# MasterBin-IIAU/UNINEXT

Hardware: NVIDIA H100
Metric: msdeformattn_fwd_bwd_gsamples_per_s (higher is better)
Workload: dtype f32

## Files before the change

### uninext_b200/csrc/msda_common.cuh

```cuda
#pragma once

#include <cuda_bf16.h>
#include <cuda_runtime.h>
#include <stdint.h>

namespace msda {

constexpr int kMaxLevels = 8;
constexpr unsigned kFullMask = 0xffffffffu;

__device__ __forceinline__ void pdl_launch_dependents() { asm volatile("griddepcontrol.launch_dependents;" ::: "memory"); }
__device__ __forceinline__ void pdl_wait_primary() { asm volatile("griddepcontrol.wait;" ::: "memory"); }

struct TapGeom {
    float lh, lw;
    int r0, r1;
    int dw;
    unsigned mask;
};

__device__ __forceinline__ TapGeom tap_geometry(float x, float y, int H, int W, int start) {
    TapGeom g;
    const float h_im = __fadd_rn(__fmul_rn(y, (float)H), -0.5f);
    const float w_im = __fadd_rn(__fmul_rn(x, (float)W), -0.5f);
    const bool inside = (h_im > -1.f) && (w_im > -1.f) && (h_im < (float)H) && (w_im < (float)W);
    const float hf = floorf(h_im), wf = floorf(w_im);
    g.lh = h_im - hf;
    g.lw = w_im - wf;
    int h0 = inside ? (int)hf : 0;
    int w0 = inside ? (int)wf : 0;
    const int h1 = h0 + 1, w1 = w0 + 1;
    unsigned m = 0;
    if (inside) {
        const bool t = h0 >= 0, b = h1 <= H - 1, l = w0 >= 0, r = w1 <= W - 1;
        m = (unsigned)(t && l) | ((unsigned)(t && r) << 1) | ((unsigned)(b && l) << 2) | ((unsigned)(b && r) << 3);
    }
    g.mask = m;
    const int ch0 = max(h0, 0), ch1 = min(h1, H - 1), cw0 = max(w0, 0), cw1 = min(w1, W - 1);
    g.r0 = start + ch0 * W + cw0;
    g.r1 = start + ch1 * W + cw0;
    g.dw = cw1 - cw0;
    return g;
}

template <typename T, int VEC> struct RowVec;

template <> struct RowVec<float, 4> {
    static constexpr int kElems = 4;
    __device__ static __forceinline__ void load(const float *p, float (&v)[4]) {
        const float4 t = __ldg(reinterpret_cast<const float4 *>(p));
        v[0] = t.x; v[1] = t.y; v[2] = t.z; v[3] = t.w;
    }
    __device__ static __forceinline__ void store(float *p, const float (&v)[4]) {
        *reinterpret_cast<float4 *>(p) = make_float4(v[0], v[1], v[2], v[3]);
    }
};

template <> struct RowVec<float, 8> {
    static constexpr int kElems = 8;
    __device__ static __forceinline__ void load(const float *p, float (&v)[8]) {
        const float4 a = __ldg(reinterpret_cast<const float4 *>(p)), b = __ldg(reinterpret_cast<const float4 *>(p) + 1);
        v[0] = a.x; v[1] = a.y; v[2] = a.z; v[3] = a.w; v[4] = b.x; v[5] = b.y; v[6] = b.z; v[7] = b.w;
    }
    __device__ static __forceinline__ void store(float *p, const float (&v)[8]) {
        reinterpret_cast<float4 *>(p)[0] = make_float4(v[0], v[1], v[2], v[3]);
        reinterpret_cast<float4 *>(p)[1] = make_float4(v[4], v[5], v[6], v[7]);
    }
};

template <> struct RowVec<__nv_bfloat16, 4> {
    static constexpr int kElems = 4;
    __device__ static __forceinline__ void load(const __nv_bfloat16 *p, float (&v)[4]) {
        const uint2 t = __ldg(reinterpret_cast<const uint2 *>(p));
        v[0] = __uint_as_float(t.x << 16); v[1] = __uint_as_float(t.x & 0xffff0000u);
        v[2] = __uint_as_float(t.y << 16); v[3] = __uint_as_float(t.y & 0xffff0000u);
    }
    __device__ static __forceinline__ void store(__nv_bfloat16 *p, const float (&v)[4]) {
        const __nv_bfloat162 a = __floats2bfloat162_rn(v[0], v[1]), b = __floats2bfloat162_rn(v[2], v[3]);
        *reinterpret_cast<uint2 *>(p) = make_uint2(*reinterpret_cast<const unsigned *>(&a),
                                                   *reinterpret_cast<const unsigned *>(&b));
    }
};

template <> struct RowVec<__nv_bfloat16, 8> {
    static constexpr int kElems = 8;
    __device__ static __forceinline__ void load(const __nv_bfloat16 *p, float (&v)[8]) {
        const uint4 t = __ldg(reinterpret_cast<const uint4 *>(p));
        const unsigned u[4] = {t.x, t.y, t.z, t.w};
#pragma unroll
        for (int i = 0; i < 4; ++i) {
            v[2 * i] = __uint_as_float(u[i] << 16);
            v[2 * i + 1] = __uint_as_float(u[i] & 0xffff0000u);
        }
    }
    __device__ static __forceinline__ void store(__nv_bfloat16 *p, const float (&v)[8]) {
        unsigned u[4];
#pragma unroll
        for (int i = 0; i < 4; ++i) {
            const __nv_bfloat162 h = __floats2bfloat162_rn(v[2 * i], v[2 * i + 1]);
            u[i] = *reinterpret_cast<const unsigned *>(&h);
        }
        *reinterpret_cast<uint4 *>(p) = make_uint4(u[0], u[1], u[2], u[3]);
    }
};

__device__ __forceinline__ void red_add_v4(float *addr, float a, float b, float c, float d) {
    asm volatile("red.global.add.v4.f32 [%0], {%1, %2, %3, %4};" ::"l"(addr), "f"(a), "f"(b), "f"(c), "f"(d) : "memory");
}

__device__ __forceinline__ void red_add_bf16x4(__nv_bfloat16 *addr, float a, float b, float c, float d) {
    const __nv_bfloat162 lo = __floats2bfloat162_rn(a, b), hi = __floats2bfloat162_rn(c, d);
    asm volatile("red.global.add.noftz.v2.bf16x2 [%0], {%1, %2};" ::"l"(addr), "r"(*reinterpret_cast<const unsigned *>(&lo)),
                 "r"(*reinterpret_cast<const unsigned *>(&hi)) : "memory");
}

__device__ __forceinline__ void red_add_mixed(bool to_bf16, __nv_bfloat16 *a16, bool to_f32, float *a32, float a, float b,
                                              float c, float d) {
    const __nv_bfloat162 lo = __floats2bfloat162_rn(a, b), hi = __floats2bfloat162_rn(c, d);
    asm volatile(
        "{\n\t.reg .pred p16, p32;\n\t"
        "setp.ne.b32 p16, %0, 0;\n\t"
        "setp.ne.b32 p32, %1, 0;\n\t"
        "@p16 red.global.add.noftz.v2.bf16x2 [%2], {%3, %4};\n\t"
        "@p32 red.global.add.v4.f32 [%5], {%6, %7, %8, %9};\n\t}"
        ::"r"((unsigned)to_bf16), "r"((unsigned)to_f32), "l"(a16), "r"(*reinterpret_cast<const unsigned *>(&lo)),
          "r"(*reinterpret_cast<const unsigned *>(&hi)), "l"(a32), "f"(a), "f"(b), "f"(c), "f"(d) : "memory");
}

}
```

### uninext_b200/csrc/msda_region.cuh

```cuda
#pragma once

#include "msda_tiled.cuh"

namespace msda {

constexpr int kRegionEdge = 8;
constexpr int kRegionHalo = 2;
constexpr int kRegionSlots = 96;
constexpr int kRegionWinRows = 1024;
constexpr int kRegionStageRows = 384;
constexpr int kRegionEntries = kRegionSlots * 16 * 4;
constexpr int kRegionTapCtas = 2;
constexpr int kRegionGvCtas = 3;
constexpr int kRegionIterSlots = kTiledWarps * 4;

using RegionTapStage = TapStage<4, 16, true>;

constexpr size_t region_tap_smem_bytes() { return (size_t)kTiledWarps * RegionTapStage::kBytes; }

constexpr size_t region_gv_smem_bytes() {
    static_assert(kRegionEntries <= 0x10000, "entry indices are u16");
    return (size_t)kRegionEntries * (4 + 2 + 2) + (size_t)kRegionSlots * 128 + (size_t)kRegionWinRows * 4;
}

#ifdef MSDA_REGION_PHASE_CLOCKS
constexpr int kRegionSpans = 4;
__device__ unsigned long long *g_region_clocks;
__device__ int g_region_knockout;
#define MSDA_REGION_CLOCK_INIT long long region_clk = clock64()
#define MSDA_REGION_CLOCK(span)                                                                  \
    if (threadIdx.x == 0) {                                                                      \
        const long long now = clock64();                                                         \
        g_region_clocks[blockIdx.x * kRegionSpans + (span)] += (unsigned long long)(now - region_clk); \
        region_clk = now;                                                                        \
    }
#define MSDA_REGION_KEEP_RED(bit) (!(g_region_knockout & (bit)))
#else
#define MSDA_REGION_CLOCK_INIT
#define MSDA_REGION_CLOCK(span)
#define MSDA_REGION_KEEP_RED(bit) true
#endif

#ifdef MSDA_REGION_COSCHED
__device__ unsigned long long *g_region_cosched[2];
__device__ __forceinline__ unsigned long long region_globaltimer() {
    unsigned long long t;
    asm volatile("mov.u64 %0, %%globaltimer;" : "=l"(t));
    return t;
}
#define MSDA_REGION_COSCHED_START(k)                                                               \
    if (threadIdx.x == 0) {                                                                        \
        unsigned smid;                                                                             \
        asm volatile("mov.u32 %0, %%smid;" : "=r"(smid));                                         \
        g_region_cosched[k][3 * blockIdx.x] = smid;                                                \
        g_region_cosched[k][3 * blockIdx.x + 1] = region_globaltimer();                            \
    }
#define MSDA_REGION_COSCHED_END(k)                                                                 \
    __syncthreads();                                                                               \
    if (threadIdx.x == 0) g_region_cosched[k][3 * blockIdx.x + 2] = region_globaltimer();
#else
#define MSDA_REGION_COSCHED_START(k)
#define MSDA_REGION_COSCHED_END(k)
#endif

struct RegionMap {
    int H[kMaxLevels], W[kMaxLevels], start[kMaxLevels];
    int Href, Wref, nry, nrx;
    int region;
    unsigned ntiles;
};

struct RegionTile {
    int b, m, nq, nwin;
    unsigned base_pair;
    int qy0[kMaxLevels], qx0[kMaxLevels], qny[kMaxLevels], qnx[kMaxLevels], qpre[kMaxLevels + 1];
    int wy0[kMaxLevels], wx0[kMaxLevels], wh[kMaxLevels], ww[kMaxLevels], wbase[kMaxLevels + 1];
};

__device__ __forceinline__ int region_first(int r, int n, int ref, int R) {
    const long long num = 2ll * r * n * R - ref;
    return num <= 0 ? 0 : (int)min((long long)n, (num + 2ll * ref - 1) / (2ll * ref));
}

template <int R, int HALO>
__global__ void __launch_bounds__(kTiledThreads, kRegionGvCtas)
msda_region_grad_value_pass(const float *__restrict__ grad_out, const int64_t *__restrict__ shapes,
                            const int64_t *__restrict__ lsi, const float *__restrict__ loc,
                            const float *__restrict__ attn, int N, int S, int M, int L, int Lq, int P, unsigned npairs,
                            float *__restrict__ grad_value)
{
    constexpr int D = 32, VEC = 4, LPR = D / VEC, GPW = 32 / LPR, LP_MAX = 16, NSL = LP_MAX / LPR;
    static_assert(GPW * kTiledWarps == kRegionIterSlots && kRegionSlots <= 256 && kRegionWinRows < 0xffff &&
                  kRegionSlots % kRegionIterSlots == 0, "entry layout");
    constexpr unsigned short kNoRow = 0xffff;

    __shared__ RegionMap rm;
    __shared__ RegionTile tl;
    __shared__ int wsum[kTiledWarps];
    __shared__ __align__(16) unsigned char slab_mem[kTiledWarps * TapSlab<LPR>::kBytes];
    extern __shared__ __align__(128) unsigned char region_dyn[];
    float *e_coef = reinterpret_cast<float *>(region_dyn);
    float4 *gstash = reinterpret_cast<float4 *>(e_coef + kRegionEntries);
    int *cnt = reinterpret_cast<int *>(gstash + kRegionSlots * LPR);
    unsigned short *e_row = reinterpret_cast<unsigned short *>(cnt + kRegionWinRows);
    unsigned short *s_idx = e_row + kRegionEntries;

    pdl_launch_dependents();
    MSDA_REGION_COSCHED_START(0);
    MSDA_REGION_CLOCK_INIT;
    if (threadIdx.x == 0) {
        int run = 0, href = 0, wref = 0;
        bool tiled = (Lq == S);
        for (int l = 0; l < L; ++l) {
            const int h = (int)shapes[2 * l], w = (int)shapes[2 * l + 1], st = (int)lsi[l];
            rm.H[l] = h; rm.W[l] = w; rm.start[l] = st;
            tiled = tiled && (st == run) && h > 0 && w > 0;
            run += h * w;
            href = max(href, h); wref = max(wref, w);
        }
        tiled = tiled && (run == S);
        rm.region = tiled ? 1 : 0;
        rm.Href = href; rm.Wref = wref;
        rm.nry = (href + R - 1) / R; rm.nrx = (wref + R - 1) / R;
        rm.ntiles = tiled ? (unsigned)N * (unsigned)M * (unsigned)(rm.nry * rm.nrx)
                          : (npairs + kRegionIterSlots - 1) / kRegionIterSlots;
    }
    __syncthreads();

    const int lane = threadIdx.x & 31, warp = threadIdx.x >> 5;
    const int sub = lane % LPR, grp = lane / LPR;
    const int LP = L * P;
    const unsigned row_elems = (unsigned)(M * D);
    TapSlab<LPR> slab(slab_mem + warp * TapSlab<LPR>::kBytes, grp);
    bool primary_done = false;
    for (unsigned tile = blockIdx.x; tile < rm.ntiles; tile += gridDim.x) {
        if (rm.region) {
            const int m = (int)(tile % (unsigned)M);
            const unsigned r = tile / (unsigned)M, per_b = (unsigned)(rm.nry * rm.nrx);
            const int reg = (int)(r % per_b), ry = reg / rm.nrx, rx = reg % rm.nrx;
            const int l = threadIdx.x;
            if (l < L) {
                const int H = rm.H[l], W = rm.W[l];
                const int y0 = region_first(ry, H, rm.Href, R), y1 = region_first(ry + 1, H, rm.Href, R);
                const int x0 = region_first(rx, W, rm.Wref, R), x1 = region_first(rx + 1, W, rm.Wref, R);
                tl.qy0[l] = y0; tl.qny[l] = y1 - y0; tl.qx0[l] = x0; tl.qnx[l] = x1 - x0;
                const int wy0 = max(0, (int)((long long)ry * R * H / rm.Href) - HALO);
                const int wy1 = min(H, (int)(((long long)(ry + 1) * R * H + rm.Href - 1) / rm.Href) + HALO);
                const int wx0 = max(0, (int)((long long)rx * R * W / rm.Wref) - HALO);
                const int wx1 = min(W, (int)(((long long)(rx + 1) * R * W + rm.Wref - 1) / rm.Wref) + HALO);
                tl.wy0[l] = wy0; tl.wh[l] = wy1 - wy0; tl.wx0[l] = wx0; tl.ww[l] = wx1 - wx0;
            }
            if (threadIdx.x == 0) { tl.m = m; tl.b = (int)(r / per_b); }
            __syncthreads();
            if (threadIdx.x == 0) {
                int nq = 0, nw = 0;
                for (int k = 0; k < L; ++k) {
                    tl.qpre[k] = nq; nq += tl.qny[k] * tl.qnx[k];
                    const int rows = tl.wh[k] * tl.ww[k];
                    if (nw + rows > kRegionWinRows) { tl.wh[k] = tl.ww[k] = 0; }
                    tl.wbase[k] = nw; nw += tl.wh[k] * tl.ww[k];
                }
                tl.qpre[L] = nq; tl.wbase[L] = nw;
                tl.nq = nq; tl.nwin = nw;
            }
        } else if (threadIdx.x == 0) {
            tl.base_pair = tile * kRegionIterSlots;
            tl.nq = (int)min((unsigned)kRegionIterSlots, npairs - tl.base_pair);
            tl.nwin = 0;
        }
        __syncthreads();
        for (int i = threadIdx.x; i < tl.nwin; i += kTiledThreads) cnt[i] = 0;
        __syncthreads();
        MSDA_REGION_CLOCK(0);

#pragma unroll 1
        for (int it = 0; it * kRegionIterSlots < tl.nq; ++it) {
            const int slot = it * kRegionIterSlots + warp * GPW + grp;
            const bool active = slot < tl.nq;
            unsigned pair = 0; int b = 0, m = 0;
            if (active) {
                if (rm.region) {
                    int l = 0;
                    while (l + 1 < L && slot >= tl.qpre[l + 1]) ++l;
                    const int k = slot - tl.qpre[l], y = tl.qy0[l] + k / tl.qnx[l], x = tl.qx0[l] + k % tl.qnx[l];
                    b = tl.b; m = tl.m;
                    pair = ((unsigned)b * (unsigned)Lq + (unsigned)(rm.start[l] + y * rm.W[l] + x)) * (unsigned)M + (unsigned)m;
                } else {
                    pair = tl.base_pair + (unsigned)slot;
                    m = (int)(pair % (unsigned)M);
                    b = (int)((pair / (unsigned)M) / (unsigned)Lq);
                }
            }
            const bool stash = rm.region && active && slot < kRegionSlots;

            float g[VEC] = {0.f, 0.f, 0.f, 0.f};
            if (active) RowVec<float, VEC>::load(grad_out + (size_t)pair * D + (size_t)sub * VEC, g);
            if (stash) gstash[slot * LPR + sub] = make_float4(g[0], g[1], g[2], g[3]);

            float4 tw[NSL];
            int2 tr[NSL];
#pragma unroll
            for (int k = 0; k < NSL; ++k) {
                const int s = sub + k * LPR;
                tw[k] = make_float4(0.f, 0.f, 0.f, 0.f);
                tr[k] = make_int2(0, 0);
                unsigned filed = 0;
                ushort4 rows4 = make_ushort4(kNoRow, kNoRow, kNoRow, kNoRow);
                float4 w4 = make_float4(0.f, 0.f, 0.f, 0.f);
                if (s < LP && active) {
                    const size_t t = (size_t)pair * LP + s;
                    const float2 xy = __ldg(reinterpret_cast<const float2 *>(loc) + t);
                    const float a = __ldg(attn + t);
                    const int l = s / P;
                    const TapGeom gm = tap_geometry(xy.x, xy.y, rm.H[l], rm.W[l], rm.start[l]);
                    w4 = masked_weights(gm, a);
                    tr[k] = make_int2(gm.r0, gm.r1 | (gm.dw << 31));
                    const unsigned nz = (unsigned)(w4.x != 0.f) | ((unsigned)(w4.y != 0.f) << 1) |
                                        ((unsigned)(w4.z != 0.f) << 2) | ((unsigned)(w4.w != 0.f) << 3);
                    if (stash) {
                        const int W = rm.W[l], o0 = gm.r0 - rm.start[l], o1 = gm.r1 - rm.start[l];
                        const int y0 = o0 / W, x0 = o0 - y0 * W, y1 = o1 / W;
                        const int wwl = tl.ww[l], whl = tl.wh[l];
                        const int ry0 = y0 - tl.wy0[l], ry1 = y1 - tl.wy0[l], rx0 = x0 - tl.wx0[l], rx1 = rx0 + gm.dw;
                        const unsigned iy0 = (unsigned)ry0 < (unsigned)whl, iy1 = (unsigned)ry1 < (unsigned)whl;
                        const unsigned ix0 = (unsigned)rx0 < (unsigned)wwl, ix1 = (unsigned)rx1 < (unsigned)wwl;
                        const unsigned inwin = (iy0 & ix0) | ((iy0 & ix1) << 1) | ((iy1 & ix0) << 2) | ((iy1 & ix1) << 3);
                        filed = inwin & nz;
                        const int w00 = tl.wbase[l] + ry0 * wwl + rx0, dhw = (y1 - y0) * wwl;
                        const int wr[4] = {w00, w00 + gm.dw, w00 + dhw, w00 + dhw + gm.dw};
#pragma unroll
                        for (int c = 0; c < 4; ++c)
                            if ((filed >> c) & 1u) atomicAdd(&cnt[wr[c]], 1);
                        rows4 = make_ushort4((filed & 1u) ? (unsigned short)wr[0] : kNoRow,
                                             (filed & 2u) ? (unsigned short)wr[1] : kNoRow,
                                             (filed & 4u) ? (unsigned short)wr[2] : kNoRow,
                                             (filed & 8u) ? (unsigned short)wr[3] : kNoRow);
                    }
                    tw[k] = make_float4((filed & 1u) ? 0.f : w4.x, (filed & 2u) ? 0.f : w4.y,
                                        (filed & 4u) ? 0.f : w4.z, (filed & 8u) ? 0.f : w4.w);
                }
                if (stash) {
                    const int e = (slot * LP_MAX + s) << 2;
                    *reinterpret_cast<ushort4 *>(e_row + e) = rows4;
                    *reinterpret_cast<float4 *>(e_coef + e) = w4;
                }
            }

            if (!primary_done) {
                pdl_wait_primary();
                primary_done = true;
            }
            const size_t slab_off = ((size_t)b * S * M + m) * D + (size_t)sub * VEC;
            float *gbase = grad_value + slab_off;
#pragma unroll
            for (int k = 0; k < NSL; ++k) {
                __syncwarp();
                slab.put(sub, tw[k], tr[k]);
                __syncwarp();
                const bool any = tw[k].x != 0.f || tw[k].y != 0.f || tw[k].z != 0.f || tw[k].w != 0.f;
                unsigned todo = (__ballot_sync(kFullMask, any) >> (grp * LPR)) & ((1u << LPR) - 1u);
                while (todo) {
                    const int j = __ffs(todo) - 1;
                    todo &= todo - 1u;
                    const float4 w4 = slab.weights(j);
                    const int2 rr = slab.rows(j);
                    const float w[4] = {w4.x, w4.y, w4.z, w4.w};
                    const unsigned dwo = (rr.y < 0) ? row_elems : 0u;
                    unsigned long long off[4];
                    off[0] = (unsigned long long)(unsigned)rr.x * row_elems;
                    off[1] = off[0] + dwo;
                    off[2] = (unsigned long long)(unsigned)(rr.y & 0x7fffffff) * row_elems;
                    off[3] = off[2] + dwo;
#pragma unroll
                    for (int c = 0; c < 4; ++c)
                        if (w[c] != 0.f && MSDA_REGION_KEEP_RED(1))
                            red_add_v4(gbase + off[c], w[c] * g[0], w[c] * g[1], w[c] * g[2], w[c] * g[3]);
                }
            }
        }

        const int nwin = tl.nwin;
        if (nwin > 0) {
            __syncthreads();
            MSDA_REGION_CLOCK(1);
            const int n = min(tl.nq, kRegionSlots) * LP_MAX * 4;
            {
                const int i0 = threadIdx.x * 4;
                int c[4], sum = 0;
#pragma unroll
                for (int q = 0; q < 4; ++q) { c[q] = (i0 + q < nwin) ? cnt[i0 + q] : 0; sum += c[q]; }
                int incl = sum;
#pragma unroll
                for (int d = 1; d < 32; d <<= 1) {
                    const int t = __shfl_up_sync(kFullMask, incl, d);
                    if (lane >= d) incl += t;
                }
                if (lane == 31) wsum[warp] = incl;
                __syncthreads();
                int run = incl - sum;
                for (int w = 0; w < warp; ++w) run += wsum[w];
#pragma unroll
                for (int q = 0; q < 4; ++q)
                    if (i0 + q < nwin) { cnt[i0 + q] = run; run += c[q]; }
            }
            static_assert(kRegionWinRows <= 4 * kTiledThreads, "scan covers 4 rows per thread");
            __syncthreads();
            for (int e = threadIdx.x; e < n; e += kTiledThreads) {
                const unsigned short r = e_row[e];
                if (r != kNoRow) s_idx[atomicAdd(&cnt[r], 1)] = (unsigned short)e;
            }
            __syncthreads();
            MSDA_REGION_CLOCK(2);

            const int b = tl.b, m = tl.m;
            for (int r = warp * GPW + grp; r < nwin; r += kRegionIterSlots) {
                const int beg = r ? cnt[r - 1] : 0, end = cnt[r];
                if (beg == end) continue;
                float4 acc = make_float4(0.f, 0.f, 0.f, 0.f);
#pragma unroll 4
                for (int i = beg; i < end; ++i) {
                    const int e = s_idx[i];
                    const float cf = e_coef[e];
                    const float4 gs = gstash[(e / (LP_MAX * 4)) * LPR + sub];
                    acc.x = fmaf(cf, gs.x, acc.x); acc.y = fmaf(cf, gs.y, acc.y);
                    acc.z = fmaf(cf, gs.z, acc.z); acc.w = fmaf(cf, gs.w, acc.w);
                }
                int l = 0;
                while (l + 1 < L && r >= tl.wbase[l + 1]) ++l;
                const int k = r - tl.wbase[l], y = tl.wy0[l] + k / tl.ww[l], x = tl.wx0[l] + k % tl.ww[l];
                const int row = rm.start[l] + y * rm.W[l] + x;
                if (MSDA_REGION_KEEP_RED(2))
                    red_add_v4(grad_value + (((size_t)b * S + row) * M + m) * D + (size_t)sub * VEC, acc.x, acc.y, acc.z, acc.w);
            }
        }
        __syncthreads();
        MSDA_REGION_CLOCK(nwin > 0 ? 3 : 1);
    }
    if (!primary_done) pdl_wait_primary();
    MSDA_REGION_COSCHED_END(0);
}

template <int R, int HALO>
__global__ void __launch_bounds__(kTiledThreads, kRegionTapCtas)
msda_bwd_region(const float *__restrict__ grad_out, const float *__restrict__ value,
                const int64_t *__restrict__ shapes, const int64_t *__restrict__ lsi,
                const float *__restrict__ loc, const float *__restrict__ attn,
                int N, int S, int M, int L, int Lq, int P, unsigned npairs, int tma,
                float *__restrict__ grad_loc, float *__restrict__ grad_attn)
{
    __shared__ WorkMap wm;
    __shared__ __align__(16) unsigned char slab_mem[kTiledWarps * TapSlab<8>::kBytes];
    __shared__ __align__(8) unsigned long long stage_bar[kTiledWarps * 2];
    extern __shared__ __align__(128) unsigned char stage_mem[];

    MSDA_REGION_COSCHED_START(1);
    if (tma)
        bwd_tiled_body<float, 4, 32, 16, true, false, false, true, false>(
            wm, slab_mem, stage_mem, stage_bar, grad_out, value, shapes, lsi, loc, attn, N, S, M, L, Lq, P, npairs, 0,
            nullptr, grad_loc, grad_attn, nullptr, 0);
    else
        bwd_tiled_body<float, 4, 32, 16, false, false, false, true, false>(
            wm, slab_mem, stage_mem, stage_bar, grad_out, value, shapes, lsi, loc, attn, N, S, M, L, Lq, P, npairs, 0,
            nullptr, grad_loc, grad_attn, nullptr, 0);
    MSDA_REGION_COSCHED_END(1);
    pdl_wait_primary();
}

struct RegionGrids {
    int gv, tap;
    size_t gv_smem;
    int gv_solo, tap_solo;
};

template <class GV, class TAP>
RegionGrids region_grids(GV gvk, size_t gv_smem, TAP tap, size_t tap_smem, int sms) {
    const auto occupancy = [](auto kern, size_t smem) {
        int per_sm = 0;
        if (cudaOccupancyMaxActiveBlocksPerMultiprocessor(&per_sm, kern, kTiledThreads, smem) != cudaSuccess || per_sm < 1)
            per_sm = 1;
        return per_sm;
    };
    const int gv_occ = occupancy(gvk, gv_smem), tap_occ = occupancy(tap, tap_smem);
    const RegionGrids solo = {gv_occ * sms, tap_occ * sms, gv_smem, gv_occ * sms, tap_occ * sms};
    int dev = 0, regs_sm = 0, smem_sm = 0, smem_optin = 0, reserved = 0, threads_sm = 0;
    cudaFuncAttributes ga{}, ta{};
    if (cudaGetDevice(&dev) != cudaSuccess ||
        cudaDeviceGetAttribute(&regs_sm, cudaDevAttrMaxRegistersPerMultiprocessor, dev) != cudaSuccess ||
        cudaDeviceGetAttribute(&smem_sm, cudaDevAttrMaxSharedMemoryPerMultiprocessor, dev) != cudaSuccess ||
        cudaDeviceGetAttribute(&smem_optin, cudaDevAttrMaxSharedMemoryPerBlockOptin, dev) != cudaSuccess ||
        cudaDeviceGetAttribute(&reserved, cudaDevAttrReservedSharedMemoryPerBlock, dev) != cudaSuccess ||
        cudaDeviceGetAttribute(&threads_sm, cudaDevAttrMaxThreadsPerMultiProcessor, dev) != cudaSuccess ||
        cudaFuncGetAttributes(&ga, gvk) != cudaSuccess || cudaFuncGetAttributes(&ta, tap) != cudaSuccess)
        return solo;
    constexpr int warps = kTiledThreads / 32;
    const auto regs = [](int per_thread) { return warps * ((per_thread * 32 + 255) / 256 * 256); };
    const auto smem = [&](const cudaFuncAttributes &a, size_t dyn) { return (long long)a.sharedSizeBytes + (long long)dyn + reserved; };
    for (int g = gv_occ; g >= 1; --g) {
        size_t dyn = gv_smem;
        if (g < gv_occ) {
            const long long over = (long long)smem_sm / (g + 1) + 1 - smem(ga, 0);
            dyn = (size_t)((over + 1023) / 1024 * 1024);
        }
        if ((long long)g * regs(ga.numRegs) + regs(ta.numRegs) <= regs_sm && (long long)dyn <= smem_optin &&
            g * smem(ga, dyn) + smem(ta, tap_smem) <= smem_sm && (g + 1) * kTiledThreads <= threads_sm) {
            if (dyn != gv_smem &&
                (cudaFuncSetAttribute(gvk, cudaFuncAttributeMaxDynamicSharedMemorySize, (int)dyn) != cudaSuccess ||
                 cudaFuncSetAttribute(gvk, cudaFuncAttributePreferredSharedMemoryCarveout,
                                      (int)cudaSharedmemCarveoutMaxShared) != cudaSuccess ||
                 occupancy(gvk, dyn) != g))
                return solo;
            return {g * sms, sms, dyn, solo.gv_solo, solo.tap_solo};
        }
    }
    return solo;
}

}
```

Baseline: 5.988.

## Replace shared-memory tap slab with warp shuffles and use 32-bit tile geometry

The grad_value kernel no longer stages each tap's weights and rows through a per-warp shared-memory slab. Each tap's scatter is now broadcast within its lane group by shuffles, inside the per-tap loop. This frees static shared memory and registers (tw/tr arrays) and drops the syncwarps. Tile-geometry arithmetic moves from 64-bit to 32-bit unsigned, guarded by a max-reference-size check, and TapGeom now carries clamped y/x coordinates so the integer divisions to recover them are gone. The carveout attribute is also now always set, which may change co-scheduling occupancy.

```diff
diff --git a/uninext_b200/csrc/msda_common.cuh b/uninext_b200/csrc/msda_common.cuh
--- a/uninext_b200/csrc/msda_common.cuh
+++ b/uninext_b200/csrc/msda_common.cuh
@@ -17,6 +17,7 @@
     int r0, r1;
     int dw;
     unsigned mask;
+    int y0, y1, x0;
 };
 
 __device__ __forceinline__ TapGeom tap_geometry(float x, float y, int H, int W, int start) {
@@ -40,6 +41,7 @@
     g.r0 = start + ch0 * W + cw0;
     g.r1 = start + ch1 * W + cw0;
     g.dw = cw1 - cw0;
+    g.y0 = ch0; g.y1 = ch1; g.x0 = cw0;
     return g;
 }
 
diff --git a/uninext_b200/csrc/msda_region.cuh b/uninext_b200/csrc/msda_region.cuh
--- a/uninext_b200/csrc/msda_region.cuh
+++ b/uninext_b200/csrc/msda_region.cuh
@@ -8,6 +8,7 @@
 constexpr int kRegionHalo = 2;
 constexpr int kRegionSlots = 96;
 constexpr int kRegionWinRows = 1024;
+constexpr int kRegionMaxRef = 1 << 15;
 constexpr int kRegionStageRows = 384;
 constexpr int kRegionEntries = kRegionSlots * 16 * 4;
 constexpr int kRegionTapCtas = 2;
@@ -78,8 +79,8 @@
 };
 
 __device__ __forceinline__ int region_first(int r, int n, int ref, int R) {
-    const long long num = 2ll * r * n * R - ref;
-    return num <= 0 ? 0 : (int)min((long long)n, (num + 2ll * ref - 1) / (2ll * ref));
+    const unsigned a = 2u * (unsigned)(r * R) * (unsigned)n;
+    return a <= (unsigned)ref ? 0 : (int)min((unsigned)n, (a + (unsigned)ref - 1u) / (2u * (unsigned)ref));
 }
 
 template <int R, int HALO>
@@ -92,12 +93,12 @@
     constexpr int D = 32, VEC = 4, LPR = D / VEC, GPW = 32 / LPR, LP_MAX = 16, NSL = LP_MAX / LPR;
     static_assert(GPW * kTiledWarps == kRegionIterSlots && kRegionSlots <= 256 && kRegionWinRows < 0xffff &&
                   kRegionSlots % kRegionIterSlots == 0, "entry layout");
+    static_assert(2ull * (kRegionMaxRef + R) * kRegionMaxRef + kRegionMaxRef < (1ull << 32), "tile geometry in 32 bits");
     constexpr unsigned short kNoRow = 0xffff;
 
     __shared__ RegionMap rm;
     __shared__ RegionTile tl;
     __shared__ int wsum[kTiledWarps];
-    __shared__ __align__(16) unsigned char slab_mem[kTiledWarps * TapSlab<LPR>::kBytes];
     extern __shared__ __align__(128) unsigned char region_dyn[];
     float *e_coef = reinterpret_cast<float *>(region_dyn);
     float4 *gstash = reinterpret_cast<float4 *>(e_coef + kRegionEntries);
@@ -118,7 +119,7 @@
             run += h * w;
             href = max(href, h); wref = max(wref, w);
         }
-        tiled = tiled && (run == S);
+        tiled = tiled && (run == S) && href <= kRegionMaxRef && wref <= kRegionMaxRef;
         rm.region = tiled ? 1 : 0;
         rm.Href = href; rm.Wref = wref;
         rm.nry = (href + R - 1) / R; rm.nrx = (wref + R - 1) / R;
@@ -131,7 +132,6 @@
     const int sub = lane % LPR, grp = lane / LPR;
     const int LP = L * P;
     const unsigned row_elems = (unsigned)(M * D);
-    TapSlab<LPR> slab(slab_mem + warp * TapSlab<LPR>::kBytes, grp);
     bool primary_done = false;
     for (unsigned tile = blockIdx.x; tile < rm.ntiles; tile += gridDim.x) {
         if (rm.region) {
@@ -144,10 +144,10 @@
                 const int y0 = region_first(ry, H, rm.Href, R), y1 = region_first(ry + 1, H, rm.Href, R);
                 const int x0 = region_first(rx, W, rm.Wref, R), x1 = region_first(rx + 1, W, rm.Wref, R);
                 tl.qy0[l] = y0; tl.qny[l] = y1 - y0; tl.qx0[l] = x0; tl.qnx[l] = x1 - x0;
-                const int wy0 = max(0, (int)((long long)ry * R * H / rm.Href) - HALO);
-                const int wy1 = min(H, (int)(((long long)(ry + 1) * R * H + rm.Href - 1) / rm.Href) + HALO);
-                const int wx0 = max(0, (int)((long long)rx * R * W / rm.Wref) - HALO);
-                const int wx1 = min(W, (int)(((long long)(rx + 1) * R * W + rm.Wref - 1) / rm.Wref) + HALO);
+                const int wy0 = max(0, (int)((unsigned)(ry * R * H) / (unsigned)rm.Href) - HALO);
+                const int wy1 = min(H, (int)((unsigned)((ry + 1) * R * H + rm.Href - 1) / (unsigned)rm.Href) + HALO);
+                const int wx0 = max(0, (int)((unsigned)(rx * R * W) / (unsigned)rm.Wref) - HALO);
+                const int wx1 = min(W, (int)((unsigned)((rx + 1) * R * W + rm.Wref - 1) / (unsigned)rm.Wref) + HALO);
                 tl.wy0[l] = wy0; tl.wh[l] = wy1 - wy0; tl.wx0[l] = wx0; tl.ww[l] = wx1 - wx0;
             }
             if (threadIdx.x == 0) { tl.m = m; tl.b = (int)(r / per_b); }
@@ -197,16 +197,13 @@
             if (active) RowVec<float, VEC>::load(grad_out + (size_t)pair * D + (size_t)sub * VEC, g);
             if (stash) gstash[slot * LPR + sub] = make_float4(g[0], g[1], g[2], g[3]);
 
-            float4 tw[NSL];
-            int2 tr[NSL];
 #pragma unroll
             for (int k = 0; k < NSL; ++k) {
                 const int s = sub + k * LPR;
-                tw[k] = make_float4(0.f, 0.f, 0.f, 0.f);
-                tr[k] = make_int2(0, 0);
                 unsigned filed = 0;
                 ushort4 rows4 = make_ushort4(kNoRow, kNoRow, kNoRow, kNoRow);
                 float4 w4 = make_float4(0.f, 0.f, 0.f, 0.f);
+                int r0 = 0, r1 = 0;
                 if (s < LP && active) {
                     const size_t t = (size_t)pair * LP + s;
                     const float2 xy = __ldg(reinterpret_cast<const float2 *>(loc) + t);
@@ -214,19 +211,17 @@
                     const int l = s / P;
                     const TapGeom gm = tap_geometry(xy.x, xy.y, rm.H[l], rm.W[l], rm.start[l]);
                     w4 = masked_weights(gm, a);
-                    tr[k] = make_int2(gm.r0, gm.r1 | (gm.dw << 31));
+                    r0 = gm.r0; r1 = gm.r1 | (gm.dw << 31);
                     const unsigned nz = (unsigned)(w4.x != 0.f) | ((unsigned)(w4.y != 0.f) << 1) |
                                         ((unsigned)(w4.z != 0.f) << 2) | ((unsigned)(w4.w != 0.f) << 3);
                     if (stash) {
-                        const int W = rm.W[l], o0 = gm.r0 - rm.start[l], o1 = gm.r1 - rm.start[l];
-                        const int y0 = o0 / W, x0 = o0 - y0 * W, y1 = o1 / W;
                         const int wwl = tl.ww[l], whl = tl.wh[l];
-                        const int ry0 = y0 - tl.wy0[l], ry1 = y1 - tl.wy0[l], rx0 = x0 - tl.wx0[l], rx1 = rx0 + gm.dw;
+                        const int ry0 = gm.y0 - tl.wy0[l], ry1 = gm.y1 - tl.wy0[l], rx0 = gm.x0 - tl.wx0[l], rx1 = rx0 + gm.dw;
                         const unsigned iy0 = (unsigned)ry0 < (unsigned)whl, iy1 = (unsigned)ry1 < (unsigned)whl;
                         const unsigned ix0 = (unsigned)rx0 < (unsigned)wwl, ix1 = (unsigned)rx1 < (unsigned)wwl;
                         const unsigned inwin = (iy0 & ix0) | ((iy0 & ix1) << 1) | ((iy1 & ix0) << 2) | ((iy1 & ix1) << 3);
                         filed = inwin & nz;
-                        const int w00 = tl.wbase[l] + ry0 * wwl + rx0, dhw = (y1 - y0) * wwl;
+                        const int w00 = tl.wbase[l] + ry0 * wwl + rx0, dhw = (ry1 - ry0) * wwl;
                         const int wr[4] = {w00, w00 + gm.dw, w00 + dhw, w00 + dhw + gm.dw};
 #pragma unroll
                         for (int c = 0; c < 4; ++c)
@@ -236,45 +231,36 @@
                                              (filed & 4u) ? (unsigned short)wr[2] : kNoRow,
                                              (filed & 8u) ? (unsigned short)wr[3] : kNoRow);
                     }
-                    tw[k] = make_float4((filed & 1u) ? 0.f : w4.x, (filed & 2u) ? 0.f : w4.y,
-                                        (filed & 4u) ? 0.f : w4.z, (filed & 8u) ? 0.f : w4.w);
                 }
                 if (stash) {
                     const int e = (slot * LP_MAX + s) << 2;
                     *reinterpret_cast<ushort4 *>(e_row + e) = rows4;
                     *reinterpret_cast<float4 *>(e_coef + e) = w4;
                 }
-            }
-
-            if (!primary_done) {
-                pdl_wait_primary();
-                primary_done = true;
-            }
-            const size_t slab_off = ((size_t)b * S * M + m) * D + (size_t)sub * VEC;
-            float *gbase = grad_value + slab_off;
-#pragma unroll
-            for (int k = 0; k < NSL; ++k) {
-                __syncwarp();
-                slab.put(sub, tw[k], tr[k]);
-                __syncwarp();
-                const bool any = tw[k].x != 0.f || tw[k].y != 0.f || tw[k].z != 0.f || tw[k].w != 0.f;
-                unsigned todo = (__ballot_sync(kFullMask, any) >> (grp * LPR)) & ((1u << LPR) - 1u);
+
+                const float4 tw = make_float4((filed & 1u) ? 0.f : w4.x, (filed & 2u) ? 0.f : w4.y,
+                                              (filed & 4u) ? 0.f : w4.z, (filed & 8u) ? 0.f : w4.w);
+                if (!primary_done) {
+                    pdl_wait_primary();
+                    primary_done = true;
+                }
+                const bool any = tw.x != 0.f || tw.y != 0.f || tw.z != 0.f || tw.w != 0.f;
+                const unsigned gmask = ((1u << LPR) - 1u) << (grp * LPR);
+                unsigned todo = (__ballot_sync(kFullMask, any) & gmask) >> (grp * LPR);
                 while (todo) {
                     const int j = __ffs(todo) - 1;
                     todo &= todo - 1u;
-                    const float4 w4 = slab.weights(j);
-                    const int2 rr = slab.rows(j);
-                    const float w[4] = {w4.x, w4.y, w4.z, w4.w};
-                    const unsigned dwo = (rr.y < 0) ? row_elems : 0u;
-                    unsigned long long off[4];
-                    off[0] = (unsigned long long)(unsigned)rr.x * row_elems;
-                    off[1] = off[0] + dwo;
-                    off[2] = (unsigned long long)(unsigned)(rr.y & 0x7fffffff) * row_elems;
-                    off[3] = off[2] + dwo;
+                    const float w[4] = {__shfl_sync(gmask, tw.x, j, LPR), __shfl_sync(gmask, tw.y, j, LPR),
+                                        __shfl_sync(gmask, tw.z, j, LPR), __shfl_sync(gmask, tw.w, j, LPR)};
+                    const int rr0 = __shfl_sync(gmask, r0, j, LPR), rr1 = __shfl_sync(gmask, r1, j, LPR);
+                    float *gbase = grad_value + ((size_t)b * S * M + m) * D + (size_t)sub * VEC;
+                    const unsigned dw = (unsigned)rr1 >> 31, r1c = (unsigned)rr1 & 0x7fffffffu;
+                    const unsigned rows[4] = {(unsigned)rr0, (unsigned)rr0 + dw, r1c, r1c + dw};
 #pragma unroll
                     for (int c = 0; c < 4; ++c)
                         if (w[c] != 0.f && MSDA_REGION_KEEP_RED(1))
-                            red_add_v4(gbase + off[c], w[c] * g[0], w[c] * g[1], w[c] * g[2], w[c] * g[3]);
+                            red_add_v4(gbase + (size_t)rows[c] * row_elems, w[c] * g[0], w[c] * g[1], w[c] * g[2],
+                                       w[c] * g[3]);
                 }
             }
         }
@@ -312,7 +298,6 @@
             __syncthreads();
             MSDA_REGION_CLOCK(2);
 
-            const int b = tl.b, m = tl.m;
             for (int r = warp * GPW + grp; r < nwin; r += kRegionIterSlots) {
                 const int beg = r ? cnt[r - 1] : 0, end = cnt[r];
                 if (beg == end) continue;
@@ -330,7 +315,8 @@
                 const int k = r - tl.wbase[l], y = tl.wy0[l] + k / tl.ww[l], x = tl.wx0[l] + k % tl.ww[l];
                 const int row = rm.start[l] + y * rm.W[l] + x;
                 if (MSDA_REGION_KEEP_RED(2))
-                    red_add_v4(grad_value + (((size_t)b * S + row) * M + m) * D + (size_t)sub * VEC, acc.x, acc.y, acc.z, acc.w);
+                    red_add_v4(grad_value + (((size_t)tl.b * S + row) * M + tl.m) * D + (size_t)sub * VEC, acc.x, acc.y, acc.z,
+                               acc.w);
             }
         }
         __syncthreads();
@@ -403,11 +389,11 @@
         }
         if ((long long)g * regs(ga.numRegs) + regs(ta.numRegs) <= regs_sm && (long long)dyn <= smem_optin &&
             g * smem(ga, dyn) + smem(ta, tap_smem) <= smem_sm && (g + 1) * kTiledThreads <= threads_sm) {
-            if (dyn != gv_smem &&
-                (cudaFuncSetAttribute(gvk, cudaFuncAttributeMaxDynamicSharedMemorySize, (int)dyn) != cudaSuccess ||
-                 cudaFuncSetAttribute(gvk, cudaFuncAttributePreferredSharedMemoryCarveout,
-                                      (int)cudaSharedmemCarveoutMaxShared) != cudaSuccess ||
-                 occupancy(gvk, dyn) != g))
+            if ((dyn != gv_smem &&
+                 cudaFuncSetAttribute(gvk, cudaFuncAttributeMaxDynamicSharedMemorySize, (int)dyn) != cudaSuccess) ||
+                cudaFuncSetAttribute(gvk, cudaFuncAttributePreferredSharedMemoryCarveout,
+                                     (int)cudaSharedmemCarveoutMaxShared) != cudaSuccess ||
+                occupancy(gvk, dyn) != g)
                 return solo;
             return {g * sms, sms, dyn, solo.gv_solo, solo.tap_solo};
         }
```

After: 6.053, median of 6. 1.1% higher.
